# rnajena/dynamont

Measured on AMD Instinct MI355X. Metric: signal samples resquiggled/sec, higher is better.
Workload: dtype f64

## Files before the change

dynamont_amd/csrc/dp_math.hpp:

```cpp
#pragma once

#include <cmath>

#if defined(__HIPCC__)
#include <hip/hip_runtime.h>
#define DYN_HD __host__ __device__ __forceinline__
#else
#define DYN_HD inline
#endif

namespace dynmath {

constexpr double NEG_INF = -__builtin_huge_val();

DYN_HD double fma_(double a, double b, double c) { return __builtin_fma(a, b, c); }

DYN_HD double max_hw(double a, double b) {
#if defined(__HIP_DEVICE_COMPILE__)
  double r;
  asm("v_max_f64 %0, %1, %2" : "=v"(r) : "v"(a), "v"(b));
  return r;
#else
  return __builtin_fmax(a, b);
#endif
}
DYN_HD double min_hw(double a, double b) {
#if defined(__HIP_DEVICE_COMPILE__)
  double r;
  asm("v_min_f64 %0, %1, %2" : "=v"(r) : "v"(a), "v"(b));
  return r;
#else
  return __builtin_fmin(a, b);
#endif
}

DYN_HD double rcp_seed(double x) {
#if defined(__HIP_DEVICE_COMPILE__)
  return __builtin_amdgcn_rcp(x);
#else
  return (double)(1.0f / (float)x);
#endif
}

DYN_HD double div_2to4(double num, double den) {
  double r = rcp_seed(den);
  double e = fma_(-den, r, 1.0);
  r = fma_(r, e, r);
  e = fma_(-den, r, 1.0);
  r = fma_(r, e, r);
  double q = num * r;
  double rem = fma_(-den, q, num);
  return fma_(rem, r, q);
}

DYN_HD double exp_nonpos(double d) {
  const double LOG2E = 0x1.71547652b82fep+0;
  const double LN2_HI = 0x1.62e42fee00000p-1;
  const double LN2_LO = 0x1.a39ef35793c76p-33;
  double kf = __builtin_rint(d * LOG2E);
  double r = fma_(-kf, LN2_HI, d);
  r = fma_(-kf, LN2_LO, r);
  double q = 0x1.af390ba7e6f47p-26;
  q = fma_(q, r, 0x1.2891d4ffbb0f9p-22);
  q = fma_(q, r, 0x1.71de0d85293b8p-19);
  q = fma_(q, r, 0x1.a019b8ca26fcfp-16);
  q = fma_(q, r, 0x1.a01a01a7cebcdp-13);
  q = fma_(q, r, 0x1.6c16c1789d1d7p-10);
  q = fma_(q, r, 0x1.11111111109a6p-7);
  q = fma_(q, r, 0x1.5555555553d37p-5);
  q = fma_(q, r, 0x1.5555555555556p-3);
  q = fma_(q, r, 0x1.0000000000001p-1);
  double p = fma_(r * r, q, r) + 1.0;
#if defined(__HIP_DEVICE_COMPILE__)
  return __builtin_amdgcn_ldexp(p, (int)kf);
#else
  return std::ldexp(p, (int)kf);
#endif
}

DYN_HD double log1p_unit(double e) {
  const double SQRT2M1 = 0x1.a827999fcef32p-2;
  const double LN2 = 0x1.62e42fefa39efp-1;
  const double c = (e > SQRT2M1) ? 1.0 : 0.0;
  const double num = e - c;
  const double den = (e + 2.0) + c;
  const double t = div_2to4(num, den);
  const double s = t * t;
  double f = 0x1.2b6686d1072f3p-4;
  f = fma_(f, s, 0x1.39fd39474ad34p-4);
  f = fma_(f, s, 0x1.7462bd8e53c17p-4);
  f = fma_(f, s, 0x1.c71c62c63e016p-4);
  f = fma_(f, s, 0x1.2492492e09d1ap-3);
  f = fma_(f, s, 0x1.9999999995204p-3);
  f = fma_(f, s, 0x1.5555555555558p-2);
  const double a = fma_(t * s, f, t);
  return fma_(c, LN2, a + a);
}

DYN_HD double softplus_nonpos(double d) {
  d = __builtin_fmax(d, -1000.0);
  return log1p_unit(exp_nonpos(d));
}

DYN_HD double log_plus(double x, double y) {
  const double hi = __builtin_fmax(x, y);
  const double lo = __builtin_fmin(x, y);
  return hi + softplus_nonpos(lo - hi);
}

struct Emis {
  double mean;
  double inv_stdev;
  double neg_log_stdev;
  double stdev;
};

constexpr double HALF_LOG_2PI = 0x1.d67f1c864beb4p-1;

DYN_HD double log_normal_pdf_exact(double x, double mean, double stdev, double log_stdev) {
  const double inv = 1.0 / stdev;
  const double diff = x - mean;
  double z = diff * inv;
  const double rem = fma_(-z, stdev, diff);
  z = fma_(rem, inv, z);
  double t = -0.5 * z;
  t = t * z;
  t = t - log_stdev;
  return t - HALF_LOG_2PI;
}

DYN_HD double log_normal_pdf(double x, const Emis& p) {
  const double z = (x - p.mean) * p.inv_stdev;
  const double t = z * z;
  return fma_(t, -0.5, p.neg_log_stdev) - HALF_LOG_2PI;
}

inline Emis make_emis(double mean, double stdev, double log_stdev) {
  Emis e;
  e.mean = mean;
  e.inv_stdev = 1.0 / stdev;
  e.neg_log_stdev = -log_stdev;
  e.stdev = stdev;
  return e;
}

struct SoftplusNode {
  double g, s;
};
constexpr int SP_STEPS = 128;
constexpr int SP_RANGE = 40;
constexpr int SP_NODES = SP_STEPS * SP_RANGE + 1;
constexpr double SP_MAGIC = 0x1.8p52;

inline void softplus_build_table(SoftplusNode* t) {
  for (int i = 0; i < SP_NODES; ++i) {
    const long double d = -(long double)i / SP_STEPS;
    const long double e = expl(d);
    t[i].g = (i == SP_NODES - 1) ? 0.0 : (double)log1pl(e);
    t[i].s = (i == SP_NODES - 1) ? 0.0 : (double)(e / (1.0L + e));
  }
}

DYN_HD double vreg_const(double c) {
#if defined(__HIP_DEVICE_COMPILE__)
  asm("" : "+v"(c));
#endif
  return c;
}

DYN_HD double sreg_const(double c) {
#if defined(__HIP_DEVICE_COMPILE__)
  asm("" : "+s"(c));
#endif
  return c;
}

DYN_HD int low_word(double m) {
#if defined(__HIP_DEVICE_COMPILE__)
  return __double2loint(m);
#else
  unsigned long long b;
  __builtin_memcpy(&b, &m, 8);
  return (int)(unsigned)(b & 0xffffffffull);
#endif
}

template <int M>
struct SoftplusLookup {
  double hi[M], r[M], g0[M], s[M];
  double diff[M];
};

template <int M>
DYN_HD void log_plus_issue(const double (&x)[M], const double (&y)[M], SoftplusLookup<M>& L,
                           const SoftplusNode* __restrict__ tab) {
#if defined(DYN_EXP_MAXPLUS)
#pragma unroll
  for (int j = 0; j < M; ++j) L.hi[j] = __builtin_fmax(x[j], y[j]);
  (void)tab;
  return;
#endif
  double d[M], m[M], kf[M];
  const double magic = vreg_const(SP_MAGIC), neg_steps = sreg_const(-(double)SP_STEPS);
#pragma unroll
  for (int j = 0; j < M; ++j) L.hi[j] = __builtin_fmax(x[j], y[j]);
#if defined(__HIP_DEVICE_COMPILE__)
#pragma unroll
  for (int j = 0; j < M; ++j) asm volatile("" : "+v"(L.hi[j]));
#endif
#pragma unroll
  for (int j = 0; j < M; ++j) L.diff[j] = x[j] - y[j];
#pragma unroll
  for (int j = 0; j < M; ++j) d[j] = __builtin_fmax(-__builtin_fabs(L.diff[j]), -(double)SP_RANGE);
#pragma unroll
  for (int j = 0; j < M; ++j) m[j] = fma_(d[j], neg_steps, magic);
#pragma unroll
  for (int j = 0; j < M; ++j) kf[j] = m[j] - magic;
#pragma unroll
  for (int j = 0; j < M; ++j) L.r[j] = fma_(kf[j], 1.0 / SP_STEPS, d[j]);
#pragma unroll
  for (int j = 0; j < M; ++j) {
    const SoftplusNode nd = tab[low_word(m[j])];
    L.g0[j] = nd.g;
    L.s[j] = nd.s;
  }
}

template <int M>
DYN_HD void log_plus_finish(const SoftplusLookup<M>& L, double (&out)[M]) {
#if defined(DYN_EXP_MAXPLUS)
#pragma unroll
  for (int j = 0; j < M; ++j) out[j] = L.hi[j];
  return;
#endif
  double u[M], w[M], p[M], q[M];
  const double c120 = vreg_const(1.0 / 120.0), c24 = vreg_const(1.0 / 24.0);
  const double m10 = sreg_const(-12.0 / 120.0), m4 = sreg_const(-0.25);
#pragma unroll
  for (int j = 0; j < M; ++j) w[j] = 1.0 - L.s[j];
#pragma unroll
  for (int j = 0; j < M; ++j) u[j] = L.s[j] * w[j];
#pragma unroll
  for (int j = 0; j < M; ++j) w[j] = w[j] - L.s[j];
#pragma unroll
  for (int j = 0; j < M; ++j) q[j] = fma_(u[j], m10, c120);
#pragma unroll
  for (int j = 0; j < M; ++j) q[j] = q[j] * w[j];
#pragma unroll
  for (int j = 0; j < M; ++j) p[j] = fma_(u[j], m4, c24);
#pragma unroll
  for (int j = 0; j < M; ++j) p[j] = fma_(q[j], L.r[j], p[j]);
#pragma unroll
  for (int j = 0; j < M; ++j) p[j] = fma_(p[j], L.r[j], w[j] * (1.0 / 6.0));
#pragma unroll
  for (int j = 0; j < M; ++j) p[j] = fma_(p[j], L.r[j], 0.5);
#pragma unroll
  for (int j = 0; j < M; ++j) u[j] = u[j] * L.r[j];
#pragma unroll
  for (int j = 0; j < M; ++j) p[j] = fma_(p[j], u[j], L.s[j]);
#pragma unroll
  for (int j = 0; j < M; ++j) out[j] = L.hi[j] + fma_(p[j], L.r[j], L.g0[j]);
}

template <int M>
DYN_HD void log_plus_finish3(const SoftplusLookup<M>& L, double (&out)[M]) {
  double u[M], w[M], p[M];
  const double c6 = sreg_const(1.0 / 6.0);
#pragma unroll
  for (int j = 0; j < M; ++j) w[j] = 1.0 - L.s[j];
#pragma unroll
  for (int j = 0; j < M; ++j) u[j] = L.s[j] * w[j];
#pragma unroll
  for (int j = 0; j < M; ++j) w[j] = w[j] - L.s[j];
#pragma unroll
  for (int j = 0; j < M; ++j) p[j] = fma_(w[j] * c6, L.r[j], 0.5);
#pragma unroll
  for (int j = 0; j < M; ++j) u[j] = u[j] * L.r[j];
#pragma unroll
  for (int j = 0; j < M; ++j) p[j] = fma_(p[j], u[j], L.s[j]);
#pragma unroll
  for (int j = 0; j < M; ++j) out[j] = L.hi[j] + fma_(p[j], L.r[j], L.g0[j]);
}

template <int M>
DYN_HD void softplus_table_vec(double (&d)[M], double (&g)[M], const SoftplusNode* __restrict__ tab) {
  double zero[M];
  SoftplusLookup<M> L;
#pragma unroll
  for (int j = 0; j < M; ++j) zero[j] = 0.0;
  log_plus_issue<M>(zero, d, L, tab);
  log_plus_finish<M>(L, g);
}
template <int M>
DYN_HD void softplus_table3_vec(double (&d)[M], double (&g)[M], const SoftplusNode* __restrict__ tab) {
  double zero[M];
  SoftplusLookup<M> L;
#pragma unroll
  for (int j = 0; j < M; ++j) zero[j] = 0.0;
  log_plus_issue<M>(zero, d, L, tab);
  log_plus_finish3<M>(L, g);
}

template <int M>
struct EmisV {
  double mean[M], inv_stdev[M], neg_log_stdev[M];
  DYN_HD void set(int j, const Emis& e) {
    mean[j] = e.mean;
    inv_stdev[j] = e.inv_stdev;
    neg_log_stdev[j] = e.neg_log_stdev;
  }
};

template <int M>
DYN_HD void log_normal_pdf_vec(double x, const EmisV<M>& p, double (&out)[M]) {
  double z[M];
#pragma unroll
  for (int j = 0; j < M; ++j) z[j] = x - p.mean[j];
#pragma unroll
  for (int j = 0; j < M; ++j) z[j] = z[j] * p.inv_stdev[j];
#pragma unroll
  for (int j = 0; j < M; ++j) z[j] = z[j] * z[j];
#pragma unroll
  for (int j = 0; j < M; ++j) z[j] = fma_(z[j], -0.5, p.neg_log_stdev[j]);
#pragma unroll
  for (int j = 0; j < M; ++j) out[j] = z[j] - HALF_LOG_2PI;
}

}
```

dynamont_amd/csrc/nt_kernels.hip:

```cpp
#include "nt_kernels.hpp"

#include <algorithm>

#include "band_runs.hpp"
#include "dp_cell.hpp"
#include "dp_math_strict.hpp"
#include "segment_kernels.hpp"

#define DYN_ONE_WAVE_PER_SIMD \
  __launch_bounds__(256 * DYN_WAVES_PER_SIMD) __attribute__((amdgpu_waves_per_eu(DYN_WAVES_PER_SIMD, DYN_WAVES_PER_SIMD)))

#define DYN_WAVES_PER_GROUP (4 * DYN_WAVES_PER_SIMD)

namespace dynk {

using dynmath::NEG_INF;
using dynmath::EmisV;
using dynmath::log_normal_pdf_vec;
using dynmath::SoftplusNode;
using dynmath::SoftplusLookup;
using dynmath::log_plus_issue;
using dynmath::log_plus_finish;
using dynmath::SP_NODES;

namespace {

typedef __attribute__((address_space(3))) uint32_t lds_u32_t;
typedef __attribute__((address_space(3))) uint64_t lds_u64_t;

__device__ __forceinline__ int pmod(int a) {
  int r = a % P;
  return r < 0 ? r + P : r;
}

__device__ __forceinline__ int pos_of(int lane, int j) { return j < 6 ? (j >> 1) * 128 + lane * 2 + (j & 1) : 384 + lane; }
__device__ __forceinline__ int row_pos(int s) { return pos_of(s / CPL, s % CPL); }

typedef double dyn_d2 __attribute__((ext_vector_type(2)));
typedef float dyn_f2 __attribute__((ext_vector_type(2)));
typedef float dyn_f4 __attribute__((ext_vector_type(4)));

template <bool NT>
__device__ __forceinline__ void store_row_f64(double* __restrict__ row, int lane, const double (&x)[CPL]) {
  static_assert(CPL == 7, "three register pairs and a single");
#pragma unroll
  for (int q = 0; q < 3; ++q) {
    dyn_d2 v;
    v.x = x[2 * q];
    v.y = x[2 * q + 1];
    dyn_d2* dst = reinterpret_cast<dyn_d2*>(row + q * 128 + lane * 2);
    if (NT) __builtin_nontemporal_store(v, dst);
    else *dst = v;
  }
  if (NT) __builtin_nontemporal_store(x[6], row + 384 + lane);
  else row[384 + lane] = x[6];
}

__device__ __forceinline__ uint64_t lanes_of_window(int c0, int len) {
  const int s0 = pmod(c0);
  const int l0 = s0 / CPL;
  const int n = (s0 + len - 1) / CPL - l0 + 1;
  if (n >= 64) return ~0ull;
  const uint64_t m = (1ull << n) - 1ull;
  return l0 ? ((m << l0) | (m >> (64 - l0))) : m;
}
__device__ __forceinline__ uint64_t uniform_u64(uint64_t v) {
  const uint32_t lo32 = (uint32_t)__builtin_amdgcn_readfirstlane((int)(uint32_t)v);
  const uint32_t hi32 = (uint32_t)__builtin_amdgcn_readfirstlane((int)(uint32_t)(v >> 32));
  return ((uint64_t)hi32 << 32) | lo32;
}
__device__ __forceinline__ uint64_t half_mask_of(uint64_t live) {
  uint64_t x = (live | (live >> 1)) & 0x5555555555555555ull;
  x = (x | (x >> 1)) & 0x3333333333333333ull;
  x = (x | (x >> 2)) & 0x0f0f0f0f0f0f0f0full;
  x = (x | (x >> 4)) & 0x00ff00ff00ff00ffull;
  x = (x | (x >> 8)) & 0x0000ffff0000ffffull;
  x = (x | (x >> 16)) & 0x00000000ffffffffull;
  return x;
}
#ifdef DYN_SKIP_OOB
constexpr bool SKIP_OOB = true;
#else
constexpr bool SKIP_OOB = false;
#endif
constexpr int OOB_SLACK = 5;

using dynband::band_mid;

__device__ __forceinline__ double readlane_f64(double v, int l) {
  int lo = __builtin_amdgcn_readlane(__double2loint(v), l);
  int hi = __builtin_amdgcn_readlane(__double2hiint(v), l);
  return __hiloint2double(hi, lo);
}

__device__ __forceinline__ double wave_ror1(double x) {
  int lo = __double2loint(x), hi = __double2hiint(x);
  const int rlo = __builtin_amdgcn_mov_dpp(lo, 0x13C, 0xf, 0xf, false);
  const int rhi = __builtin_amdgcn_mov_dpp(hi, 0x13C, 0xf, 0xf, false);
  return __hiloint2double(rhi, rlo);
}

__device__ __forceinline__ double wave_rol1(double x) {
  int lo = __double2loint(x), hi = __double2hiint(x);
  const int rlo = __builtin_amdgcn_mov_dpp(lo, 0x134, 0xf, 0xf, false);
  const int rhi = __builtin_amdgcn_mov_dpp(hi, 0x134, 0xf, 0xf, false);
  return __hiloint2double(rhi, rlo);
}

__device__ __forceinline__ void from_left(const double (&x)[CPL], double (&out)[CPL]) {
  out[0] = wave_ror1(x[CPL - 1]);
#pragma unroll
  for (int j = 1; j < CPL; ++j) out[j] = x[j - 1];
}

__device__ __forceinline__ void from_right(const double (&x)[CPL], double (&out)[CPL]) {
#pragma unroll
  for (int j = 0; j < CPL - 1; ++j) out[j] = x[j + 1];
  out[CPL - 1] = wave_rol1(x[0]);
}

__device__ __forceinline__ Emis load_emis(const Emis* __restrict__ pr, int n, int N) {
  Emis e;
  if (n >= 1 && n < N) {
    e = pr[n - 1];
  } else {
    e.mean = 0.0;
    e.inv_stdev = 1.0;
    e.neg_log_stdev = NEG_INF;
    e.stdev = 1.0;
  }
  return e;
}

struct WaveCtx {
  int lane;
  lds_u32_t* pt;
  int log_r;
};

struct RowCursor {
  int page = -1;
  uint32_t base = 0;
  __device__ __forceinline__ uint32_t at(const WaveCtx& w, int t) {
    const int pg = t >> w.log_r;
    if (pg != page) {
      page = pg;
      base = (uint32_t)__builtin_amdgcn_readfirstlane((int)w.pt[pg]) << w.log_r;
    }
    return base + ((uint32_t)t & ((1u << w.log_r) - 1u));
  }
};

__device__ __forceinline__ uint32_t pool_row(const WaveCtx& w, int t) {
  return (w.pt[t >> w.log_r] << w.log_r) + ((uint32_t)t & ((1u << w.log_r) - 1u));
}

__device__ __forceinline__ void wave_lds_sync() {
  __builtin_amdgcn_fence(__ATOMIC_ACQ_REL, "workgroup");
  __builtin_amdgcn_wave_barrier();
}
__device__ __forceinline__ void wave_lds_sync_local() {
  __builtin_amdgcn_fence(__ATOMIC_ACQ_REL, "workgroup", "local");
  __builtin_amdgcn_wave_barrier();
}

constexpr int RING_D = DYN_WAVES_PER_SIMD == 1 ? 4 : 2;
constexpr int ROW_BYTES = P * 8;
constexpr int RING_WAIT = 4 * (RING_D - 1);

#define DYN_DMA_MOD " nt"
__device__ __forceinline__ void ring_dma_row(const double* row_lane_ptr, unsigned lds_slot_addr) {
  asm volatile(
      "s_mov_b32 m0, %1\n\t"
      "s_nop 0\n\t"
      "global_load_lds_dwordx4 %0, off" DYN_DMA_MOD "\n\t"
      "global_load_lds_dwordx4 %0, off offset:1024" DYN_DMA_MOD "\n\t"
      "global_load_lds_dwordx4 %0, off offset:2048" DYN_DMA_MOD "\n\t"
      "s_mov_b32 exec_hi, 0\n\t"
      "global_load_lds_dwordx4 %0, off offset:3072" DYN_DMA_MOD "\n\t"
      "s_mov_b32 exec_hi, -1\n\t"
      ::"v"(row_lane_ptr), "s"(__builtin_amdgcn_readfirstlane(lds_slot_addr))
      : "memory");
}

__device__ __forceinline__ void ring_dma_row_masked(const double* row_lane_ptr, unsigned lds_slot_addr, uint64_t live, uint64_t half) {
  asm volatile(
      "s_mov_b32 m0, %1\n\t"
      "s_mov_b64 exec, %2\n\t"
      "global_load_lds_dwordx4 %0, off" DYN_DMA_MOD "\n\t"
      "global_load_lds_dwordx4 %0, off offset:1024" DYN_DMA_MOD "\n\t"
      "global_load_lds_dwordx4 %0, off offset:2048" DYN_DMA_MOD "\n\t"
      "s_mov_b64 exec, %3\n\t"
      "global_load_lds_dwordx4 %0, off offset:3072" DYN_DMA_MOD "\n\t"
      "s_mov_b64 exec, -1\n\t"
      ::"v"(row_lane_ptr), "s"(__builtin_amdgcn_readfirstlane(lds_slot_addr)), "s"(live), "s"(half)
      : "memory");
}

template <int N>
__device__ __forceinline__ void wait_vmcnt() {
  asm volatile("s_waitcnt vmcnt(%0)" ::"n"(N) : "memory");
}

__device__ __forceinline__ void ring_read_row(unsigned slot_addr, int lane, double (&b)[CPL]) {
  static_assert(CPL == 7, "ring_read_row is written for 7 cells per lane");
  dyn_d2 p0, p1, p2;
  double last;
  asm volatile(
      "ds_read_b128 %0, %4\n\t"
      "ds_read_b128 %1, %4 offset:1024\n\t"
      "ds_read_b128 %2, %4 offset:2048\n\t"
      "ds_read_b64 %3, %5 offset:3072\n\t"
      "s_waitcnt lgkmcnt(0)"
      : "=&v"(p0), "=&v"(p1), "=&v"(p2), "=&v"(last)
      : "v"(slot_addr + lane * 16), "v"(slot_addr + lane * 8)
      : "memory");
  b[0] = p0.x;
  b[1] = p0.y;
  b[2] = p1.x;
  b[3] = p1.y;
  b[4] = p2.x;
  b[5] = p2.y;
  b[6] = last;
}

template <bool STORE, int ARITH>
__device__ __forceinline__ double backward_sweep(const ReadDesc& rd, const WaveCtx& w,
                                                 const double* __restrict__ sig,
                                                 const Emis* __restrict__ par, double* __restrict__ ws,
                                                 double m1, double e2, const SoftplusNode* s_tab, uint32_t* fallbacks = nullptr) {
  const int lane = w.lane;
  uint32_t nfb = 0;
  const int T = (int)rd.T, N = (int)rd.N, bw = (int)rd.bw, W = 2 * bw + 1;
  const double ratio = rd.ratio;
  const double* __restrict__ sg = sig + rd.sig_off;
  const Emis* __restrict__ pr = par + rd.par_off;
  double* __restrict__ out = ws;
  RowCursor cur;

  bool bad_sample = false;
  int lo = band_mid(T - 1, ratio) - bw;
  const double inv_ratio = 1.0 / ratio;
  constexpr bool MASKED = SKIP_OOB && STORE && ARITH != ARITH_FOLDED;
  uint64_t store_mask = MASKED ? uniform_u64(lanes_of_window(lo - OOB_SLACK, W + 2 * OOB_SLACK)) : ~0ull;
  const int n_init = lo + bw;
  int n[CPL];
  double bE[CPL], bM[CPL], bE2[CPL], bM2[CPL], e[CPL];
  EmisV<CPL> p;
  double p_stdev[ARITH == ARITH_STRICT ? CPL : 1];
  double p_ylo[ARITH == ARITH_STRICT ? CPL : 1];
  auto set_p = [&](int j, const Emis& em) {
    set_emis<ARITH>(p, j, em);
    if constexpr (ARITH == ARITH_STRICT) {
      p_stdev[j] = em.stdev;
      p_ylo[j] = dynmath::recip_lo(em.stdev, em.inv_stdev);
    }
  };
  constexpr double SAMPLE_MAX = ARITH == ARITH_STRICT ? 1e300 : 1.7976931348623157e308;
  {
    const size_t rT = STORE ? (size_t)cur.at(w, T) * P : 0, rT1 = STORE ? (size_t)cur.at(w, T - 1) * P : 0;
#pragma unroll
    for (int j = 0; j < CPL; ++j) {
      const int slot = lane * CPL + j;
      n[j] = lo + pmod(slot - lo);
      set_p(j, load_emis(pr, n[j], (n[j] <= lo + W - 1) ? N : 0));
      bE[j] = (n[j] == n_init) ? 0.0 : NEG_INF;
      bM[j] = NEG_INF;
    }
    if (STORE) {
      store_row_f64<false>(out + rT1, lane, bE);
      store_row_f64<false>(out + rT, lane, bM);
    }
  }

  for (int thi = T - 2; thi >= 0; thi -= 64) {
    const int base = thi - 63;
    const int idx = base + lane;
    const double xs = (idx >= 0) ? sg[idx] : 0.0;
    bad_sample |= !(fabs(xs) <= SAMPLE_MAX);
    const int ilo = base < 0 ? -base : 0;
    emission_vec<ARITH>(readlane_f64(xs, 63), p, p_stdev, p_ylo, e);
    auto hand_over = [&](int new_lo) {
      const int leaving = lo + P - 1;
      const int top = lo + W - 1;
      const Emis fresh = load_emis(pr, new_lo, N);
      const Emis none = load_emis(pr, 0, 0);
#pragma unroll
      for (int j = 0; j < CPL; ++j) {
        if (n[j] == leaving) {
          n[j] = new_lo;
          set_p(j, fresh);
        }
        if (n[j] == top) {
          bE[j] = NEG_INF;
          set_p(j, none);
        }
      }
      lo = new_lo;
      if constexpr (MASKED) store_mask = uniform_u64(lanes_of_window(lo - OOB_SLACK, W + 2 * OOB_SLACK));
    };
    auto row = [&](int t, const double (&bE_in)[CPL], const double (&bM_in)[CPL], double (&bE_out)[CPL], double (&bM_out)[CPL]) {
      const int i = t - base;
      double Y[CPL], Yr[CPL], x1[CPL], x2[CPL];
#pragma unroll
      for (int j = 0; j < CPL; ++j) Y[j] = bM_in[j] + e[j];
#pragma unroll
      for (int j = 0; j < CPL; ++j) bM_out[j] = bE_in[j] + e[j];
      from_right(Y, Yr);
#pragma unroll
      for (int j = 0; j < CPL; ++j) x1[j] = Yr[j] + m1;
#pragma unroll
      for (int j = 0; j < CPL; ++j) x2[j] = bM_out[j] + e2;
      SoftplusLookup<CPL> L;
      log_plus_issue<CPL>(x1, x2, L, s_tab);
      {
        const double xnext = readlane_f64(xs, i > 0 ? i - 1 : 0);
        emission_vec<ARITH>(xnext, p, p_stdev, p_ylo, e);
      }
      if constexpr (ARITH == ARITH_FOLDED) dynmath::log_plus_finish3<CPL>(L, bE_out);
      else if constexpr (ARITH == ARITH_STRICT) log_plus_finish_certified(L, bE_out, strict_tab(s_tab), nfb);
      else log_plus_finish<CPL>(L, bE_out);
      const size_t rt = STORE ? (size_t)cur.at(w, t) * P : 0;
      if constexpr (STORE && ARITH == ARITH_FOLDED) {
        double ls[CPL];
#pragma unroll
        for (int j = 0; j < CPL; ++j) ls[j] = x2[j] - bE_out[j];
        store_row_f64<true>(out + rt, lane, ls);
      } else if (STORE) {
        if constexpr (MASKED) {
          if (__builtin_amdgcn_inverse_ballot_w64(store_mask)) store_row_f64<true>(out + rt, lane, bE_out);
        } else {
          store_row_f64<true>(out + rt, lane, bE_out);
        }
      }
    };
    int t = thi;
    const int tlo = base + ilo;
#pragma unroll 1
    while (t >= tlo) {
      const int new_lo = band_mid(t, ratio) - bw;
      if (new_lo != lo) hand_over(new_lo);
      const int tq = __builtin_amdgcn_readfirstlane(dynband::run_first_row(t, ratio, inv_ratio, tlo));
#pragma unroll 1
      for (; t - 1 >= tq; t -= 2) {
        row(t, bE, bM, bE2, bM2);
        row(t - 1, bE2, bM2, bE, bM);
      }
      if (t >= tq) {
        row(t, bE, bM, bE2, bM2);
#pragma unroll
        for (int j = 0; j < CPL; ++j) {
          bE[j] = bE2[j];
          bM[j] = bM2[j];
        }
        --t;
      }
    }
  }
  const bool any_bad = __any(bad_sample);
  if (ARITH == ARITH_STRICT && fallbacks) *fallbacks += nfb;
  return any_bad ? NEG_INF : readlane_f64(bE[0], 0);
}

__device__ __forceinline__ double max_f64(double a, double b) {
  double r;
  asm("v_max_f64 %0, %1, %2" : "=v"(r) : "v"(a), "v"(b));
  return r;
}

template <bool POST, bool INPLACE, bool STRICT>
__device__ __forceinline__ double forward_sweep(const ReadDesc& rd, const WaveCtx& w,
                                                const double* __restrict__ sig, const Emis* __restrict__ par,
                                                const double* __restrict__ ws_rd, float* __restrict__ lp_out,
                                                uint64_t* __restrict__ bits, double Z, double m1, double e2,
                                                const SoftplusNode* s_tab, unsigned ring_base, int strict_rows = 0,
                                                uint32_t* fallbacks = nullptr) {
  uint32_t nfb = 0;
  const int lane = w.lane;
  const int T = (int)rd.T, N = (int)rd.N, bw = (int)rd.bw, W = 2 * bw + 1;
  const double ratio = rd.ratio;
  const double* __restrict__ sg = sig + rd.sig_off;
  const Emis* __restrict__ pr = par + rd.par_off;
  const double* __restrict__ lat = ws_rd;
  float* __restrict__ lat_lp = lp_out;
  RowCursor cur_dma, cur_out;

  int lo = band_mid(1, ratio) - bw;
  const double inv_ratio = 1.0 / ratio;
  constexpr bool MASKED = SKIP_OOB && POST;
  uint64_t dma_mask = ~0ull, dma_half = 0xffffffffull, out_mask = ~0ull;
  auto set_masks = [&]() {
    if constexpr (MASKED) {
      dma_mask = uniform_u64(lanes_of_window(lo, W + OOB_SLACK));
      dma_half = half_mask_of(dma_mask);
      out_mask = uniform_u64(lanes_of_window(lo - 1, W + 1));
    }
  };
  set_masks();
  if constexpr (MASKED) {
    auto* ringp = (__attribute__((address_space(3))) double*)(size_t)ring_base;
#pragma unroll
    for (int k = 0; k < RING_D * P / 64; ++k) ringp[k * 64 + lane] = NEG_INF;
    wave_lds_sync_local();
  }
  int n[CPL];
  struct RowState {
    double fM[CPL], fE[CPL], e[CPL], vM[CPL], vE[CPL], b[CPL];
  };
  RowState sa, sb;
  EmisV<CPL> p;
  double p_stdev[STRICT ? CPL : 1];
  double p_ylo[STRICT ? CPL : 1];
  auto set_p = [&](int j, const Emis& e, auto with_stdev) {
    if constexpr (!POST) set_emis<ARITH_FOLDED>(p, j, e);
    else p.set(j, e);
    if constexpr (STRICT && decltype(with_stdev)::value) {
      p_stdev[j] = e.stdev;
      p_ylo[j] = dynmath::recip_lo(e.stdev, e.inv_stdev);
    }
  };
  auto emission = [&](bool strict_row, double x, double (&out)[CPL]) {
    if constexpr (STRICT) {
      if (strict_row) {
#ifdef DYN_QUOT5
        dynmath::log_normal_pdf_cert_vec<CPL>(x, p, p_stdev, out);
#else
        dynmath::log_normal_pdf_cert4_vec<CPL>(x, p, p_stdev, p_ylo, out);
#endif
        return;
      }
    }
    if constexpr (!POST) emission_vec<ARITH_FOLDED>(x, p, p_stdev, p_ylo, out);
    else log_normal_pdf_vec<CPL>(x, p, out);
  };
  const double x0 = sg[0];
  const size_t r1 = POST ? (size_t)cur_out.at(w, 1) * P : 0;
#pragma unroll
  for (int j = 0; j < CPL; ++j) {
    const int slot = lane * CPL + j;
    n[j] = lo + pmod(slot - lo);
    set_p(j, load_emis(pr, n[j], (n[j] <= lo + W - 1) ? N : 0), std::true_type{});
    sa.fE[j] = (n[j] == 0) ? 0.0 : NEG_INF;
    sa.fM[j] = NEG_INF;
    sa.vE[j] = sa.fE[j];
    sa.vM[j] = NEG_INF;
    sa.b[j] = POST ? lat[r1 + pos_of(lane, j)] : NEG_INF;
  }
  emission(1 <= strict_rows, x0, sa.e);
  const double* __restrict__ dma_src = ws_rd + lane * 2;
  if (POST) {
    for (int r = 2; r <= RING_D + 1; ++r) {
      if constexpr (MASKED) ring_dma_row_masked(dma_src + (size_t)cur_dma.at(w, min(r, T)) * P, ring_base + (r % RING_D) * ROW_BYTES, dma_mask, dma_half);
      else ring_dma_row(dma_src + (size_t)cur_dma.at(w, min(r, T)) * P, ring_base + (r % RING_D) * ROW_BYTES);
    }
  }

  auto hand_over = [&](auto strict_tag, int next_lo) {
    const Emis none = load_emis(pr, 0, 0);
    const Emis entering = load_emis(pr, lo + W, N);
#pragma unroll
    for (int j = 0; j < CPL; ++j) {
      const bool leaves = n[j] == lo;
      n[j] = leaves ? lo + P : n[j];
      if (leaves) set_p(j, none, strict_tag);
      if (n[j] == lo + W) set_p(j, entering, strict_tag);
    }
    lo = next_lo;
    set_masks();
  };

  auto row = [&](auto strict_tag, int t, double xn, const RowState& in, RowState& out) {
    constexpr bool STRICT_ROW = STRICT && decltype(strict_tag)::value;
    double fEl[CPL], vEl[CPL];
    if (POST) {
      wait_vmcnt<RING_WAIT>();
      ring_read_row(ring_base + ((t + 1) % RING_D) * ROW_BYTES, lane, out.b);
      if constexpr (MASKED)
        ring_dma_row_masked(dma_src + (size_t)cur_dma.at(w, min(t + 1 + RING_D, T)) * P, ring_base + ((t + 1) % RING_D) * ROW_BYTES, dma_mask, dma_half);
      else
        ring_dma_row(dma_src + (size_t)cur_dma.at(w, min(t + 1 + RING_D, T)) * P, ring_base + ((t + 1) % RING_D) * ROW_BYTES);
    }
    from_left(in.fE, fEl);
    if (POST) from_left(in.vE, vEl);
    double a1[CPL], a2[CPL];
#pragma unroll
    for (int j = 0; j < CPL; ++j) out.fM[j] = (fEl[j] + in.e[j]) + m1;
#pragma unroll
    for (int j = 0; j < CPL; ++j) a1[j] = in.fM[j] + in.e[j];
#pragma unroll
    for (int j = 0; j < CPL; ++j) a2[j] = (in.fE[j] + in.e[j]) + e2;
    if constexpr (STRICT_ROW) {
      SoftplusLookup<CPL> L;
      log_plus_issue<CPL>(a1, a2, L, s_tab);
      emission(true, xn, out.e);
      log_plus_finish_certified(L, out.fE, strict_tab(s_tab), nfb);
    } else {
      SoftplusLookup<CPL> L;
      log_plus_issue<CPL>(a1, a2, L, s_tab);
      emission(false, xn, out.e);
      if constexpr (!POST) dynmath::log_plus_finish3<CPL>(L, out.fE);
      else log_plus_finish<CPL>(L, out.fE);
    }
    if (POST) {
      double LPM[CPL], LPE[CPL], alt[CPL];
      uint64_t bj[CPL];
#pragma unroll
      for (int j = 0; j < CPL; ++j) LPM[j] = (out.fM[j] + (out.b[j] + out.e[j])) - Z;
#pragma unroll
      for (int j = 0; j < CPL; ++j) LPE[j] = (out.fE[j] + in.b[j]) - Z;
#pragma unroll
      for (int j = 0; j < CPL; ++j) out.vM[j] = vEl[j] + LPM[j];
#pragma unroll
      for (int j = 0; j < CPL; ++j) out.vE[j] = max_f64(in.vM[j], in.vE[j]) + LPE[j];
#pragma unroll
      for (int j = 0; j < CPL; ++j) alt[j] = in.vM[j] + LPE[j];
#pragma unroll
      for (int j = 0; j < CPL; ++j) bj[j] = __ballot(out.vE[j] == alt[j]);
      unsigned wlo, whi;
      static_assert(CPL == 7, "one v_writelane pair per cell register");
#define DYN_WL(J, LO, HI) "v_writelane_b32 %0, %" #LO ", " #J "\n\tv_writelane_b32 %1, %" #HI ", " #J "\n\t"
      asm("s_nop 4\n\t"
          DYN_WL(0, 2, 3) DYN_WL(1, 4, 5) DYN_WL(2, 6, 7) DYN_WL(3, 8, 9) DYN_WL(4, 10, 11) DYN_WL(5, 12, 13) DYN_WL(6, 14, 15)
          : "=&v"(wlo), "=&v"(whi)
          : "s"((unsigned)bj[0]), "s"((unsigned)(bj[0] >> 32)), "s"((unsigned)bj[1]), "s"((unsigned)(bj[1] >> 32)),
            "s"((unsigned)bj[2]), "s"((unsigned)(bj[2] >> 32)), "s"((unsigned)bj[3]), "s"((unsigned)(bj[3] >> 32)),
            "s"((unsigned)bj[4]), "s"((unsigned)(bj[4] >> 32)), "s"((unsigned)bj[5]), "s"((unsigned)(bj[5] >> 32)),
            "s"((unsigned)bj[6]), "s"((unsigned)(bj[6] >> 32)));
#undef DYN_WL
      const uint64_t mybits = ((uint64_t)whi << 32) | wlo;
      const uint32_t prow = cur_out.at(w, t);
      const size_t rt = (size_t)prow * P;
      const bool out_live = MASKED ? __builtin_amdgcn_inverse_ballot_w64(out_mask) : true;
      if (!out_live) {
      } else if (INPLACE) {
#pragma unroll
        for (int q = 0; q < 3; ++q) {
          dyn_f4 v4;
          v4.x = (float)LPM[2 * q];
          v4.y = (float)LPE[2 * q];
          v4.z = (float)LPM[2 * q + 1];
          v4.w = (float)LPE[2 * q + 1];
          __builtin_nontemporal_store(v4, reinterpret_cast<dyn_f4*>(&lat_lp[2 * (rt + q * 128 + lane * 2)]));
        }
        dyn_f2 v2;
        v2.x = (float)LPM[6];
        v2.y = (float)LPE[6];
        __builtin_nontemporal_store(v2, reinterpret_cast<dyn_f2*>(&lat_lp[2 * (rt + 384 + lane)]));
      } else {
#pragma unroll
        for (int q = 0; q < 3; ++q) {
          dyn_f2 v2;
          v2.x = (float)LPE[2 * q];
          v2.y = (float)LPE[2 * q + 1];
          __builtin_nontemporal_store(v2, reinterpret_cast<dyn_f2*>(&lat_lp[rt + q * 128 + lane * 2]));
        }
        __builtin_nontemporal_store((float)LPE[6], &lat_lp[rt + 384 + lane]);
      }
      if (lane < CPL) bits[(size_t)prow * CPL + lane] = mybits;
    }
  };

  auto block = [&](auto strict_tag, int tb) {
    const int idx = tb + lane;
    const double xs = (idx < T - 1) ? sg[idx] : 0.0;
    asm volatile("" ::"v"(xs));
    const int tend = tb + min(64, T - tb);
    int t = tb;
#pragma unroll 1
    while (t < tend) {
      const int next_lo = band_mid(t + 1, ratio) - bw;
      if (next_lo != lo) hand_over(strict_tag, next_lo);
      const int te = __builtin_amdgcn_readfirstlane(dynband::next_move_row(t + 1, ratio, inv_ratio, tend));
#pragma unroll 1
      for (; t + 1 < te; t += 2) {
        row(strict_tag, t, readlane_f64(xs, t - tb), sa, sb);
        row(strict_tag, t + 1, readlane_f64(xs, t + 1 - tb), sb, sa);
      }
      if (t < te) {
        row(strict_tag, t, readlane_f64(xs, t - tb), sa, sb);
        sa = sb;
        ++t;
      }
    }
  };
  int tb = 1;
  if constexpr (STRICT) {
    for (; tb < T && tb <= strict_rows; tb += 64) block(std::true_type{}, tb);
  }
  for (; tb < T; tb += 64) block(std::false_type{}, tb);
  const double (&fE)[CPL] = sa.fE;
  if (STRICT && fallbacks) *fallbacks += nfb;
  if (POST) wait_vmcnt<0>();
  const int nf = band_mid(T - 1, ratio);
  const int sf = pmod(nf);
  double zf = 0.0;
#pragma unroll
  for (int j = 0; j < CPL; ++j)
    if (j == sf % CPL) zf = fE[j];
  return readlane_f64(zf, sf / CPL);
}

__device__ __forceinline__ bool z_ok(const ReadDesc& rd, double Zf, double Zb) {
  const double size = (double)((uint64_t)rd.T * (uint64_t)(2 * rd.bw + 3));
  if (isinf(Zf) || isinf(Zb)) return false;
  return !(fabs(Zf - Zb) / size > 1e-8);
}

__device__ __forceinline__ bool traceback(const ReadDesc& rd, const WaveCtx& w, const float* __restrict__ lp,
                                          const uint64_t* __restrict__ bits, TraceBuffers tb, bool inplace,
                                          lds_u64_t* sb) {
  const int lane = w.lane;
  const int T = (int)rd.T, N = (int)rd.N;
  double* __restrict__ pp = tb.pp + rd.path_off;
  uint32_t* __restrict__ pathn = tb.pathn + rd.path_off;
  uint32_t* __restrict__ segrow = tb.segrow + rd.seg_off;

  int t = T - 1, n = N - 1;
  int slot = n % P;
  int stM = 0;
#ifndef DYN_EXP_TB_SERIAL
  uint64_t nb[CPL];
  uint32_t nprow = 0;
  auto fetch = [&](int base_) {
    const int row_ = base_ + lane;
    nprow = 0;
#pragma unroll
    for (int j = 0; j < CPL; ++j) nb[j] = 0;
    if (row_ >= 1) {
      nprow = pool_row(w, row_);
#pragma unroll
      for (int j = 0; j < CPL; ++j) nb[j] = bits[(size_t)nprow * CPL + j];
    }
  };
  int pend_row = 0, pend_n = 0, pend_st = -1;
  float pend_lp = 0.0f;
  auto finish = [&]() {
    if (pend_st >= 0) {
      if (inplace || pend_st == 0) pp[pend_row] = exp((double)pend_lp);
      pathn[pend_row] = (uint32_t)pend_n | (pend_st ? 0x80000000u : 0u);
      if (pend_st) segrow[pend_n - 1] = (uint32_t)pend_row;
    }
    pend_st = -1;
  };
  int sj = slot % CPL, sq = slot / CPL;
  if (t > 0 && n > 0) fetch(t - 63);
  while (t > 0 && n > 0) {
    const int base = t - 63;
    const int row = base + lane;
    const uint32_t prow = nprow;
#pragma unroll
    for (int j = 0; j < CPL; ++j) sb[lane * CPL + j] = nb[j];
    wave_lds_sync_local();
    if (base > 1) fetch(base - 64);
    int my_n = 0, my_st = -1;
    const int block_lo = base < 1 ? 1 : base;
    const uint64_t in_block = base >= 1 ? ~0ull : (~0ull << (1 - base));
    while (t >= block_lo && n > 0) {
      const int tl = t - base;
      if (stM) {
        if (__builtin_amdgcn_inverse_ballot_w64(1ull << tl)) {
          my_n = n;
          my_st = 1;
        }
        --n;
        if (sj == 0) {
          sj = CPL - 1;
          sq = sq ? sq - 1 : 63;
        } else {
          --sj;
        }
        stM = 0;
        --t;
        continue;
      }
      const uint64_t wd = sb[lane * CPL + sj];
      const uint64_t upto = (2ull << tl) - 1ull;
      const uint64_t m = __ballot((wd >> sq) & 1) & upto & in_block;
      if (m) {
        const int rl = 63 - __builtin_clzll(m);
        if (__builtin_amdgcn_inverse_ballot_w64(upto & ~((1ull << rl) - 1ull))) {
          my_n = n;
          my_st = 0;
        }
        if (base + rl - 1 >= block_lo) {
          if (__builtin_amdgcn_inverse_ballot_w64(1ull << (rl - 1))) {
            my_n = n;
            my_st = 1;
          }
          --n;
          if (sj == 0) {
            sj = CPL - 1;
            sq = sq ? sq - 1 : 63;
          } else {
            --sj;
          }
          t = base + rl - 2;
        } else {
          t = base + rl - 1;
          stM = 1;
        }
      } else {
        if (__builtin_amdgcn_inverse_ballot_w64(upto & in_block)) {
          my_n = n;
          my_st = 0;
        }
        t = block_lo - 1;
      }
    }
    finish();
    if (my_st >= 0) {
      const size_t cell = (size_t)prow * P + row_pos(my_n % P);
      if (inplace) pend_lp = lp[2 * cell + (my_st ? 0 : 1)];
      else if (my_st == 0) pend_lp = lp[cell];
      pend_row = row;
      pend_n = my_n;
      pend_st = my_st;
    }
    wave_lds_sync_local();
  }
  finish();
#else
  while (t > 0 && n > 0) {
    const int base = t - 63;
    const int row = base + lane;
    uint32_t prow = 0;
    if (row >= 1) {
      prow = pool_row(w, row);
#pragma unroll
      for (int j = 0; j < CPL; ++j) sb[lane * CPL + j] = bits[(size_t)prow * CPL + j];
    }
    wave_lds_sync();
    int my_n = 0, my_slot = 0, my_st = -1;
    const int block_lo = base < 1 ? 1 : base;
    while (t >= block_lo && n > 0) {
      if (stM) {
        if (row == t) {
          my_n = n;
          my_slot = slot;
          my_st = 1;
        }
        --n;
        slot = slot ? slot - 1 : P - 1;
        stM = 0;
        --t;
        continue;
      }
      const uint64_t wd = sb[lane * CPL + (slot % CPL)];
      const bool bit = (row >= block_lo) && (row <= t) && ((wd >> (slot / CPL)) & 1);
      const uint64_t m = __ballot(bit);
      const int r = m ? base + (63 - __builtin_clzll(m)) : block_lo - 1;
      const int e_lo = m ? r : block_lo;
      if (row >= e_lo && row <= t) {
        my_n = n;
        my_slot = slot;
        my_st = 0;
      }
      if (m) {
        t = r - 1;
        stM = 1;
      } else {
        t = block_lo - 1;
      }
    }
    if (my_st >= 0) {
      const size_t cell = (size_t)prow * P + row_pos(my_slot);
      if (inplace) pp[row] = exp((double)lp[2 * cell + (my_st ? 0 : 1)]);
      else if (my_st == 0) pp[row] = exp((double)lp[cell]);
      pathn[row] = (uint32_t)my_n | (my_st ? 0x80000000u : 0u);
      if (my_st) segrow[my_n - 1] = (uint32_t)row;
    }
    wave_lds_sync();
  }
#endif
  return t == 0 && n == 0;
}

__device__ __forceinline__ void mpost(const ReadDesc& rd, const WaveCtx& w, const double* __restrict__ bE,
                                      const float* __restrict__ lp, const double* __restrict__ sig,
                                      const Emis* __restrict__ par, TraceBuffers tb, double Zb, double m1) {
  const int T = (int)rd.T, N = (int)rd.N;
  const double* __restrict__ sg = sig + rd.sig_off;
  for (int n = 1 + w.lane; n < N; n += 64) {
    const int row = (int)tb.segrow[rd.seg_off + n - 1];
    const int slot = n % P, pslot = (n - 1) % P;
    double fE_prev;
    if (row == 1) {
      fE_prev = n == 1 ? 0.0 : NEG_INF;
    } else {
      const size_t pcell = (size_t)pool_row(w, row - 1) * P + row_pos(pslot);
      fE_prev = ((double)lp[pcell] - bE[pcell]) + Zb;
    }
    const Emis em = par[rd.par_off + n - 1];
    const double e_here = dynmath::log_normal_pdf(sg[row - 1], em);
    const double e_next = row + 1 < T ? dynmath::log_normal_pdf(sg[row], em) : NEG_INF;
    const double fM = (fE_prev + e_here) + m1;
    const double bM = bE[(size_t)pool_row(w, row + 1) * P + row_pos(slot)] + e_next;
    tb.pp[rd.path_off + row] = exp((fM + bM) - Zb);
  }
}

__device__ __forceinline__ double forward_train_chain(const ReadDesc& rd, const WaveCtx& w, const double* __restrict__ sig,
                                                      const double* __restrict__ ws, TrainBuffers tb, double Zb,
                                                      const SoftplusNode* s_tab, unsigned ring_base) {
  const int lane = w.lane;
  const int T = (int)rd.T, N = (int)rd.N, bw = (int)rd.bw;
  const double ratio = rd.ratio;
  const double* __restrict__ sg = sig + rd.sig_off;
  double* __restrict__ cw = tb.col_w + rd.par_off;
  double* __restrict__ cs1 = tb.col_s1 + rd.par_off;
  double* __restrict__ cs2 = tb.col_s2 + rd.par_off;
  const double* __restrict__ etab = exp128_tab(s_tab);
  RowCursor cur_dma;

  int lo = band_mid(1, ratio) - bw;
  double gE[CPL], gM[CPL];
  double aw[CPL], a1[CPL], a2[CPL];
  double awsum = 0.0;
#pragma unroll
// ... 751 lines not shown
```

Baseline: 548.4.

## Pipeline LDS softplus lookups and ring reads across cell groups in posterior sweep

In the non-strict posterior row, the seven softplus table lookups are split into groups of 1+2+2+2 cells. Each group's LDS reads are issued as raw ds_read_b128 instructions with partial lgkmcnt waits, so the emission computation and the LPE/vE work on earlier cells can overlap with later lookups. The ring-buffer LDS read is now issued early and waited on only at the end. The DMA refill is moved to target the slot the previous row consumed, which lowers the number of rows prefetched ahead, and the vmcnt wait is loosened to match. This interleaving depends on manual waitcnt counting and asm operand constraints, and getting either wrong could cause hazards. The shallower prefetch could also expose more global latency.

```diff
diff --git a/dynamont_amd/csrc/dp_math.hpp b/dynamont_amd/csrc/dp_math.hpp
--- a/dynamont_amd/csrc/dp_math.hpp
+++ b/dynamont_amd/csrc/dp_math.hpp
@@ -192,35 +192,48 @@
 };
 
 template <int M>
+DYN_HD void log_plus_index(const double (&x)[M], const double (&y)[M], SoftplusLookup<M>& L, int (&k)[M]) {
+#if defined(DYN_EXP_MAXPLUS)
+#pragma unroll
+  for (int j = 0; j < M; ++j) L.hi[j] = __builtin_fmax(x[j], y[j]);
+#pragma unroll
+  for (int j = 0; j < M; ++j) k[j] = 0;
+  return;
+#endif
+  double d[M], m[M], kf[M];
+  const double magic = vreg_const(SP_MAGIC), neg_steps = sreg_const(-(double)SP_STEPS);
+#pragma unroll
+  for (int j = 0; j < M; ++j) L.hi[j] = __builtin_fmax(x[j], y[j]);
+#if defined(__HIP_DEVICE_COMPILE__)
+#pragma unroll
+  for (int j = 0; j < M; ++j) asm volatile("" : "+v"(L.hi[j]));
+#endif
+#pragma unroll
+  for (int j = 0; j < M; ++j) L.diff[j] = x[j] - y[j];
+#pragma unroll
+  for (int j = 0; j < M; ++j) d[j] = __builtin_fmax(-__builtin_fabs(L.diff[j]), -(double)SP_RANGE);
+#pragma unroll
+  for (int j = 0; j < M; ++j) m[j] = fma_(d[j], neg_steps, magic);
+#pragma unroll
+  for (int j = 0; j < M; ++j) kf[j] = m[j] - magic;
+#pragma unroll
+  for (int j = 0; j < M; ++j) L.r[j] = fma_(kf[j], 1.0 / SP_STEPS, d[j]);
+#pragma unroll
+  for (int j = 0; j < M; ++j) k[j] = low_word(m[j]);
+}
+
+template <int M>
 DYN_HD void log_plus_issue(const double (&x)[M], const double (&y)[M], SoftplusLookup<M>& L,
                            const SoftplusNode* __restrict__ tab) {
+  int k[M];
+  log_plus_index<M>(x, y, L, k);
 #if defined(DYN_EXP_MAXPLUS)
-#pragma unroll
-  for (int j = 0; j < M; ++j) L.hi[j] = __builtin_fmax(x[j], y[j]);
   (void)tab;
   return;
 #endif
-  double d[M], m[M], kf[M];
-  const double magic = vreg_const(SP_MAGIC), neg_steps = sreg_const(-(double)SP_STEPS);
-#pragma unroll
-  for (int j = 0; j < M; ++j) L.hi[j] = __builtin_fmax(x[j], y[j]);
-#if defined(__HIP_DEVICE_COMPILE__)
-#pragma unroll
-  for (int j = 0; j < M; ++j) asm volatile("" : "+v"(L.hi[j]));
-#endif
-#pragma unroll
-  for (int j = 0; j < M; ++j) L.diff[j] = x[j] - y[j];
-#pragma unroll
-  for (int j = 0; j < M; ++j) d[j] = __builtin_fmax(-__builtin_fabs(L.diff[j]), -(double)SP_RANGE);
-#pragma unroll
-  for (int j = 0; j < M; ++j) m[j] = fma_(d[j], neg_steps, magic);
-#pragma unroll
-  for (int j = 0; j < M; ++j) kf[j] = m[j] - magic;
-#pragma unroll
-  for (int j = 0; j < M; ++j) L.r[j] = fma_(kf[j], 1.0 / SP_STEPS, d[j]);
 #pragma unroll
   for (int j = 0; j < M; ++j) {
-    const SoftplusNode nd = tab[low_word(m[j])];
+    const SoftplusNode nd = tab[k[j]];
     L.g0[j] = nd.g;
     L.s[j] = nd.s;
   }
diff --git a/dynamont_amd/csrc/nt_kernels.hip b/dynamont_amd/csrc/nt_kernels.hip
--- a/dynamont_amd/csrc/nt_kernels.hip
+++ b/dynamont_amd/csrc/nt_kernels.hip
@@ -197,9 +197,38 @@
       : "memory");
 }
 
+constexpr int RING_WAIT_LATE = 4 * (RING_D - 2);
+static_assert(RING_D >= 2, "forward_sweep refills the slot the previous row read");
+
 template <int N>
 __device__ __forceinline__ void wait_vmcnt() {
   asm volatile("s_waitcnt vmcnt(%0)" ::"n"(N) : "memory");
+}
+
+struct RingRow {
+  dyn_d2 p0, p1, p2;
+  double last;
+};
+__device__ __forceinline__ void ring_read_issue(unsigned slot_addr, int lane, RingRow& r) {
+  asm volatile(
+      "ds_read_b128 %0, %4\n\t"
+      "ds_read_b128 %1, %4 offset:1024\n\t"
+      "ds_read_b128 %2, %4 offset:2048\n\t"
+      "ds_read_b64 %3, %5 offset:3072"
+      : "=&v"(r.p0), "=&v"(r.p1), "=&v"(r.p2), "=&v"(r.last)
+      : "v"(slot_addr + lane * 16), "v"(slot_addr + lane * 8)
+      : "memory");
+}
+#define DYN_RING_ROW_OPERANDS(R) "+v"((R).p0), "+v"((R).p1), "+v"((R).p2), "+v"((R).last)
+__device__ __forceinline__ void ring_row_landed(const RingRow& r, double (&b)[CPL]) {
+  static_assert(CPL == 7, "a ring row is read for 7 cells per lane");
+  b[0] = r.p0.x;
+  b[1] = r.p0.y;
+  b[2] = r.p1.x;
+  b[3] = r.p1.y;
+  b[4] = r.p2.x;
+  b[5] = r.p2.y;
+  b[6] = r.last;
 }
 
 __device__ __forceinline__ void ring_read_row(unsigned slot_addr, int lane, double (&b)[CPL]) {
@@ -368,6 +397,40 @@
   return r;
 }
 
+template <int M>
+struct LookupGroup {
+  SoftplusLookup<M> L;
+  dyn_d2 nd[M];
+};
+template <int J0, int M>
+__device__ __forceinline__ void lp_issue_cells(const double (&x)[CPL], const double (&y)[CPL], LookupGroup<M>& G, unsigned tab_addr) {
+  double xs[M], ys[M];
+  int k[M];
+#pragma unroll
+  for (int i = 0; i < M; ++i) {
+    xs[i] = x[J0 + i];
+    ys[i] = y[J0 + i];
+  }
+  dynmath::log_plus_index<M>(xs, ys, G.L, k);
+#if !defined(DYN_EXP_MAXPLUS)
+#pragma unroll
+  for (int i = 0; i < M; ++i) asm volatile("ds_read_b128 %0, %1" : "=v"(G.nd[i]) : "v"(tab_addr + 16u * (unsigned)k[i]));
+#endif
+}
+template <int J0, int M>
+__device__ __forceinline__ void lp_finish_cells(LookupGroup<M>& G, double (&out)[CPL]) {
+  double o[M];
+#pragma unroll
+  for (int i = 0; i < M; ++i) {
+    G.L.g0[i] = G.nd[i].x;
+    G.L.s[i] = G.nd[i].y;
+  }
+  log_plus_finish<M>(G.L, o);
+#pragma unroll
+  for (int i = 0; i < M; ++i) out[J0 + i] = o[i];
+}
+#define DYN_LGKM_WAIT(N, ...) asm volatile("s_waitcnt lgkmcnt(" #N ")" : __VA_ARGS__)
+
 template <bool POST, bool INPLACE, bool STRICT>
 __device__ __forceinline__ double forward_sweep(const ReadDesc& rd, const WaveCtx& w,
                                                 const double* __restrict__ sig, const Emis* __restrict__ par,
@@ -449,7 +512,7 @@
   emission(1 <= strict_rows, x0, sa.e);
   const double* __restrict__ dma_src = ws_rd + lane * 2;
   if (POST) {
-    for (int r = 2; r <= RING_D + 1; ++r) {
+    for (int r = 2; r <= RING_D; ++r) {
       if constexpr (MASKED) ring_dma_row_masked(dma_src + (size_t)cur_dma.at(w, min(r, T)) * P, ring_base + (r % RING_D) * ROW_BYTES, dma_mask, dma_half);
       else ring_dma_row(dma_src + (size_t)cur_dma.at(w, min(r, T)) * P, ring_base + (r % RING_D) * ROW_BYTES);
     }
@@ -472,13 +535,18 @@
   auto row = [&](auto strict_tag, int t, double xn, const RowState& in, RowState& out) {
     constexpr bool STRICT_ROW = STRICT && decltype(strict_tag)::value;
     double fEl[CPL], vEl[CPL];
+    RingRow rb;
     if (POST) {
-      wait_vmcnt<RING_WAIT>();
-      ring_read_row(ring_base + ((t + 1) % RING_D) * ROW_BYTES, lane, out.b);
+      wait_vmcnt<RING_WAIT_LATE>();
+      ring_read_issue(ring_base + ((t + 1) % RING_D) * ROW_BYTES, lane, rb);
       if constexpr (MASKED)
-        ring_dma_row_masked(dma_src + (size_t)cur_dma.at(w, min(t + 1 + RING_D, T)) * P, ring_base + ((t + 1) % RING_D) * ROW_BYTES, dma_mask, dma_half);
+        ring_dma_row_masked(dma_src + (size_t)cur_dma.at(w, min(t + RING_D, T)) * P, ring_base + (t % RING_D) * ROW_BYTES, dma_mask, dma_half);
       else
-        ring_dma_row(dma_src + (size_t)cur_dma.at(w, min(t + 1 + RING_D, T)) * P, ring_base + ((t + 1) % RING_D) * ROW_BYTES);
+        ring_dma_row(dma_src + (size_t)cur_dma.at(w, min(t + RING_D, T)) * P, ring_base + (t % RING_D) * ROW_BYTES);
+      if constexpr (STRICT_ROW) {
+        DYN_LGKM_WAIT(0, DYN_RING_ROW_OPERANDS(rb));
+        ring_row_landed(rb, out.b);
+      }
     }
     from_left(in.fE, fEl);
     if (POST) from_left(in.vE, vEl);
@@ -489,31 +557,56 @@
     for (int j = 0; j < CPL; ++j) a1[j] = in.fM[j] + in.e[j];
 #pragma unroll
     for (int j = 0; j < CPL; ++j) a2[j] = (in.fE[j] + in.e[j]) + e2;
+    double LPM[CPL], LPE[CPL], alt[CPL];
+    auto post_e = [&](auto j0, auto cnt) {
+#pragma unroll
+      for (int j = j0; j < j0 + cnt; ++j) LPE[j] = (out.fE[j] + in.b[j]) - Z;
+#pragma unroll
+      for (int j = j0; j < j0 + cnt; ++j) out.vE[j] = max_f64(in.vM[j], in.vE[j]) + LPE[j];
+#pragma unroll
+      for (int j = j0; j < j0 + cnt; ++j) alt[j] = in.vM[j] + LPE[j];
+    };
     if constexpr (STRICT_ROW) {
       SoftplusLookup<CPL> L;
       log_plus_issue<CPL>(a1, a2, L, s_tab);
       emission(true, xn, out.e);
       log_plus_finish_certified(L, out.fE, strict_tab(s_tab), nfb);
-    } else {
+    } else if constexpr (!POST) {
       SoftplusLookup<CPL> L;
       log_plus_issue<CPL>(a1, a2, L, s_tab);
       emission(false, xn, out.e);
-      if constexpr (!POST) dynmath::log_plus_finish3<CPL>(L, out.fE);
-      else log_plus_finish<CPL>(L, out.fE);
+      dynmath::log_plus_finish3<CPL>(L, out.fE);
+    } else {
+      static_assert(CPL == 7, "1 + 2 + 2 + 2 cells");
+      const unsigned tab_addr = (unsigned)(size_t)(__attribute__((address_space(3))) const SoftplusNode*)s_tab;
+      LookupGroup<1> G0;
+      LookupGroup<2> G1, G3, G5;
+      lp_issue_cells<0, 1>(a1, a2, G0, tab_addr);
+      lp_issue_cells<1, 2>(a1, a2, G1, tab_addr);
+      double xe = xn;
+      asm volatile("" : "+s"(xe));
+      emission(false, xe, out.e);
+      DYN_LGKM_WAIT(2, "+v"(G0.nd[0]), "+v"(out.e[0]), "+v"(out.e[1]), "+v"(out.e[2]), "+v"(out.e[3]), "+v"(out.e[4]), "+v"(out.e[5]), "+v"(out.e[6]));
+      lp_finish_cells<0, 1>(G0, out.fE);
+      lp_issue_cells<3, 2>(a1, a2, G3, tab_addr);
+      DYN_LGKM_WAIT(2, "+v"(G1.nd[0]), "+v"(G1.nd[1]), "+v"(out.fE[0]));
+      lp_finish_cells<1, 2>(G1, out.fE);
+      lp_issue_cells<5, 2>(a1, a2, G5, tab_addr);
+      DYN_LGKM_WAIT(2, "+v"(G3.nd[0]), "+v"(G3.nd[1]), "+v"(out.fE[1]), "+v"(out.fE[2]));
+      lp_finish_cells<3, 2>(G3, out.fE);
+      post_e(std::integral_constant<int, 0>{}, std::integral_constant<int, 5>{});
+      DYN_LGKM_WAIT(0, "+v"(G5.nd[0]), "+v"(G5.nd[1]), "+v"(alt[0]), "+v"(alt[1]), "+v"(alt[2]), "+v"(alt[3]), "+v"(alt[4]), DYN_RING_ROW_OPERANDS(rb));
+      ring_row_landed(rb, out.b);
+      lp_finish_cells<5, 2>(G5, out.fE);
+      post_e(std::integral_constant<int, 5>{}, std::integral_constant<int, 2>{});
     }
     if (POST) {
-      double LPM[CPL], LPE[CPL], alt[CPL];
       uint64_t bj[CPL];
+      if constexpr (STRICT_ROW) post_e(std::integral_constant<int, 0>{}, std::integral_constant<int, CPL>{});
 #pragma unroll
       for (int j = 0; j < CPL; ++j) LPM[j] = (out.fM[j] + (out.b[j] + out.e[j])) - Z;
 #pragma unroll
-      for (int j = 0; j < CPL; ++j) LPE[j] = (out.fE[j] + in.b[j]) - Z;
-#pragma unroll
       for (int j = 0; j < CPL; ++j) out.vM[j] = vEl[j] + LPM[j];
-#pragma unroll
-      for (int j = 0; j < CPL; ++j) out.vE[j] = max_f64(in.vM[j], in.vE[j]) + LPE[j];
-#pragma unroll
-      for (int j = 0; j < CPL; ++j) alt[j] = in.vM[j] + LPE[j];
 #pragma unroll
       for (int j = 0; j < CPL; ++j) bj[j] = __ballot(out.vE[j] == alt[j]);
       unsigned wlo, whi;
```

Result: slower. 541.4 (-1.3%).
